# ElesionKyrie/Extreme-Video-Compression-With-Prediction-Using-Pre-trainded-Diffusion-Models-

Measured on AMD Instinct MI355X. Metric: decoded frames/sec (128x128x30) at q3, higher is better.
Workload: dtype f32

## Files before the change

extreme-video-compression-with-prediction-using-pre-trainded-diffusion-models-_amd/build.py:

```python
import os
import shutil
import subprocess
import sys
from concurrent.futures import ThreadPoolExecutor

HERE = os.path.dirname(os.path.abspath(__file__))
CSRC = os.path.join(HERE, "csrc")
LIBDIR = os.path.join(HERE, "lib")
OBJDIR = os.path.join(HERE, "build")
INCLUDE = os.path.join(os.path.dirname(HERE), "include")
HIP_SOURCES = ["conv_igemm.hip", "attention.hip", "norm.hip", "fir.hip", "elementwise.hip", "gdn.hip", "stride2.hip", "lpips.hip", "i3d.hip", "frames.hip", "noise.hip", "yuv.hip", "rate.hip", "ssim.hip", "api.hip"]
ARCH = "gfx950"


def _newer(target, deps):
    if not os.path.exists(target):
        return True
    t = os.path.getmtime(target)
    return any(os.path.getmtime(d) > t for d in deps)


def _run(cmd):
    r = subprocess.run(cmd, capture_output=True, text=True)
    if r.returncode != 0:
        raise RuntimeError("build failed: %s\n%s\n%s" % (" ".join(cmd), r.stdout, r.stderr))


def hipcc_path():
    for c in (os.environ.get("HIPCC"), shutil.which("hipcc"), "/opt/rocm/bin/hipcc"):
        if c and os.path.exists(c):
            return c
    raise RuntimeError("hipcc not found (ROCm toolchain required to build libevc_hip.so)")


def build(force=False, verbose=False):
    os.makedirs(LIBDIR, exist_ok=True)
    os.makedirs(OBJDIR, exist_ok=True)
    headers = [os.path.join(INCLUDE, h) for h in ("evc_hip.h", "evc_rans.h")]
    hipcc = hipcc_path()
    flags = ["--offload-arch=" + ARCH, "-O3", "-std=c++17", "-fPIC", "-I", INCLUDE]
    flags += os.environ.get("EVC_HIPCC_FLAGS", "").split()

    def compile_one(src):
        s = os.path.join(CSRC, src)
        o = os.path.join(OBJDIR, src.replace(".hip", ".o"))
        if force or _newer(o, [s] + headers):
            if verbose:
                print("hipcc", src, flush=True)
            _run([hipcc] + flags + ["-c", s, "-o", o])
        return o

    with ThreadPoolExecutor(max_workers=min(6, len(HIP_SOURCES))) as ex:
        objs = list(ex.map(compile_one, HIP_SOURCES))
    hip_so = os.path.join(LIBDIR, "libevc_hip.so")
    if force or _newer(hip_so, objs):
        _run([hipcc, "--offload-arch=" + ARCH, "-shared", "-fPIC", "-o", hip_so] + objs)
    rans_src = os.path.join(CSRC, "rans.cpp")
    rans_so = os.path.join(LIBDIR, "libevc_rans.so")
    if force or _newer(rans_so, [rans_src] + headers):
        _run([shutil.which("g++") or "g++", "-O2", "-std=c++17", "-fPIC", "-shared", "-Wall", "-I", INCLUDE,
              rans_src, "-o", rans_so])
    return hip_so, rans_so


# ... 3 lines not shown
```

extreme-video-compression-with-prediction-using-pre-trainded-diffusion-models-_amd/lib.py:

```python
import ctypes
import os
from ctypes import POINTER, c_char_p, c_double, c_float, c_int, c_int32, c_longlong, c_uint, c_uint8, c_ulonglong, c_void_p

import numpy as np
import torch

HERE = os.path.dirname(os.path.abspath(__file__))
HIP_SO = os.path.join(HERE, "lib", "libevc_hip.so")
if os.environ.get("EVC_HIP_SO"):
    HIP_SO = os.path.abspath(os.environ["EVC_HIP_SO"])
RANS_SO = os.path.join(HERE, "lib", "libevc_rans.so")

ACT_NONE, ACT_SILU, ACT_RELU = 0, 1, 2
ARITH_F32, ARITH_BF16X6, ARITH_F16X3 = 0, 1, 2
_ARITH_NAMES = {"f32": ARITH_F32, "bf16x6": ARITH_BF16X6, "f16x3": ARITH_F16X3}
_ARITH_DTYPES = {ARITH_F32: torch.float32, ARITH_BF16X6: torch.bfloat16, ARITH_F16X3: torch.float16}


def _arith_policy():
    name = os.environ.get("EVC_CONV_ARITH", "f16x3").lower()
    if name not in _ARITH_NAMES:
        raise ValueError(f"EVC_CONV_ARITH must be one of {sorted(_ARITH_NAMES)}, got {name!r}")
    return _ARITH_NAMES[name]

# ... 61 lines not shown
                                  c_void_p]),
    "evc_gn_coeffs_bound_f32": (c_int, [c_void_p, c_int, c_int, c_void_p, c_int, c_int, c_int, c_int, c_int, c_float,
                                        c_int, c_void_p, c_void_p, c_void_p, c_int, c_void_p, c_void_p, c_void_p,
                                        c_void_p, c_void_p, c_void_p]),
    "evc_moments_bound_f32": (c_int, [c_void_p, c_int, c_int, c_int, c_int, c_int, c_int, c_void_p, c_void_p, c_void_p]),
    "evc_gn_coeffs_site_f32": (c_int, [c_void_p, c_int, c_int, c_void_p, c_int, c_int, c_int, c_int, c_int, c_float,
                                       c_int, c_void_p, c_void_p, c_void_p, c_int, c_void_p, c_void_p, c_void_p,
                                       c_void_p, c_void_p, c_int, c_void_p]),
    "evc_gn_coeffs_bound_site_f32": (c_int, [c_void_p, c_int, c_int, c_void_p, c_int, c_int, c_int, c_int, c_int, c_float,
                                             c_int, c_void_p, c_void_p, c_void_p, c_int, c_void_p, c_void_p, c_void_p,
                                             c_void_p, c_void_p, c_void_p, c_int, c_void_p]),
    "evc_moments_bound_site_f32": (c_int, [c_void_p, c_int, c_int, c_int, c_int, c_int, c_int, c_void_p, c_void_p, c_void_p,
                                           c_int, c_void_p]),
    "evc_invariant_plan_revision": (c_int, []),
    "evc_conv_plan_query": (c_int, [POINTER(ConvArgs), POINTER(ConvPlan)]),
    "evc_gn_coeffs_bound_sample_f32": (c_int, [c_void_p, c_int, c_int, c_void_p, c_int, c_int, c_int, c_int, c_int, c_float,
                                               c_int, c_void_p, c_void_p, c_void_p, c_int, c_void_p, c_void_p, c_void_p,
                                               c_void_p, c_void_p, c_void_p, c_int, c_void_p]),
    "evc_moments_bound_sample_f32": (c_int, [c_void_p, c_int, c_int, c_int, c_int, c_int, c_int, c_void_p, c_void_p, c_void_p,
                                             c_int, c_void_p]),
    "evc_attention_invariant_workspace_bytes": (c_longlong, [c_int, c_int, c_int, c_int]),
    "evc_attention_invariant_f32": (c_int, [c_void_p, c_void_p, c_void_p, c_int, c_void_p, c_int, c_int, c_int, c_int, c_int,
                                            c_float, c_void_p, c_void_p, c_void_p]),
    "evc_attention_f16x3_f32": (c_int, [c_void_p, c_void_p, c_void_p, c_int, c_void_p, c_int, c_int, c_int, c_int, c_int,
                                        c_float, c_void_p, c_void_p, c_void_p]),
    "evc_deconv5x5s2_phase_weights_f32": (c_int, [c_void_p, c_void_p, c_int, c_int, c_int, c_int, c_void_p]),
    "evc_conv5x5s2_phase_weights_f32": (c_int, [c_void_p, c_void_p, c_int, c_int, c_int, c_void_p]),
    "evc_depth_to_space2_f32": (c_int, [c_void_p, c_int, c_int, c_void_p, c_int, c_int, c_int, c_int, c_void_p]),
    "evc_space_to_depth2_f32": (c_int, [c_void_p, c_int, c_int, c_void_p, c_int, c_int, c_int, c_int, c_int, c_void_p]),
    "evc_deconv5x5s2_workspace_bytes": (c_longlong, [c_int, c_int, c_int, c_int]),
    "evc_deconv5x5s2_f32": (c_int, [c_void_p, c_void_p, c_int, c_void_p, c_void_p, c_void_p] + [c_int] * 6 + [c_void_p]),
    "evc_conv5x5s2_workspace_bytes": (c_longlong, [c_int, c_int, c_int, c_int]),
    "evc_conv5x5s2_f32": (c_int, [c_void_p, c_int, c_void_p, c_int, c_void_p, c_void_p, c_void_p] + [c_int] * 6 + [c_void_p]),
    "evc_gdn_workspace_bytes": (c_longlong, [c_int, c_int, c_int, c_int]),
    "evc_gdn_f32": (c_int, [c_void_p, c_void_p, c_int, c_void_p, c_void_p, c_void_p, c_int, c_int, c_int, c_int, c_int,
                            c_int, c_void_p]),
    "evc_affine_act_nhwc_f32": (c_int, [c_void_p, c_void_p, c_void_p, c_void_p, c_int, c_int, c_int, c_int, c_int,
                                        c_int, c_void_p]),
    "evc_conv_co_pad": (c_int, [c_int]),
    "evc_conv_packed_floats": (c_longlong, [c_int, c_int, c_int, c_int]),
    "evc_conv_pack_weights_f32": (c_int, [c_void_p, c_void_p, c_int, c_int, c_int, c_int, c_void_p]),
    "evc_conv_packed_bytes": (c_longlong, [c_int, c_int, c_int, c_int, c_int]),
    "evc_conv_pack_weights": (c_int, [c_void_p, c_void_p, c_int, c_int, c_int, c_int, c_int, c_void_p]),
    "evc_conv_set_option": (c_int, [c_char_p, c_int]),
    "evc_spade_act_nhwc_f32": (c_int, [c_void_p, c_void_p, c_void_p, c_void_p, c_int, c_void_p, c_void_p, c_int, c_void_p,
                                       c_void_p, c_int, c_void_p, c_int, c_int, c_int, c_int, c_int, c_void_p]),
    "evc_conv_choose_splits": (c_int, [POINTER(ConvArgs)]),
    "evc_conv_kernel_name": (c_int, [POINTER(ConvArgs), c_char_p, c_int]),
    "evc_conv_fused_1x1_supported": (c_int, [POINTER(ConvArgs)]),
    "evc_conv_stats_splits": (c_int, [POINTER(ConvArgs)]),
    "evc_conv_workspace_bytes": (c_longlong, [POINTER(ConvArgs)]),
    "evc_conv2d_nhwc_f32": (c_int, [POINTER(ConvArgs), c_void_p, c_void_p]),
    "evc_conv2d_nhwc_profiled_f32": (c_int, [POINTER(ConvArgs), c_void_p, c_void_p, c_void_p, c_void_p]),
    "evc_attention_f32": (c_int, [c_void_p, c_void_p, c_void_p, c_int, c_void_p, c_int, c_int, c_int, c_int, c_int,
                                  c_float, c_void_p]),
    "evc_attention_workspace_bytes": (c_longlong, [c_int, c_int, c_int, c_int]),
    "evc_attention_set_option": (c_int, [c_char_p, c_int]),
    "evc_attention_ws_f32": (c_int, [c_void_p, c_void_p, c_void_p, c_int, c_void_p, c_int, c_int, c_int, c_int, c_int,
                                     c_float, c_void_p, c_void_p]),
    "evc_frame_group_norm_f32": (c_int, [c_void_p] * 4 + [c_int] * 5 + [c_float, c_void_p]),
    "evc_frame_attention_f32": (c_int, [c_void_p, c_int, c_void_p, c_int] + [c_int] * 5 + [c_float, c_void_p]),
    "evc_frame_mix_f32": (c_int, [c_void_p] * 4 + [c_int] * 3 + [c_longlong, c_void_p]),
    "evc_frame_taps_f32": (c_int, [c_void_p, c_void_p] + [c_int] * 4 + [c_void_p]),
    "evc_ddpm_step_f32": (c_int, [c_void_p, c_void_p, c_void_p, c_longlong] + [c_float] * 5 + [c_int, c_void_p]),
    "evc_ddim_step_f32": (c_int, [c_void_p, c_void_p, c_longlong] + [c_float] * 4 + [c_int, c_void_p]),
    "evc_axpy_f32": (c_int, [c_void_p, c_void_p, c_void_p, c_longlong, c_float, c_void_p]),
    "evc_pndm_transfer_f32": (c_int, [c_void_p, c_void_p, c_void_p, c_longlong, c_float, c_float, c_float, c_int,
                                      c_void_p]),
    "evc_lincomb4_f32": (c_int, [c_void_p] * 5 + [c_longlong] + [c_float] * 4 + [c_void_p]),
    "evc_scale_clamp_f32": (c_int, [c_void_p, c_void_p, c_longlong, c_float, c_float, c_int, c_float, c_float,
                                    c_void_p]),
    "evc_gate_residual_f32": (c_int, [c_void_p, c_void_p, c_void_p, c_void_p, c_longlong, c_void_p]),
    "evc_elic_gather_params_f32": (c_int, [c_void_p] + [c_int] * 8 + [c_void_p, c_int, c_void_p, c_void_p,
                                                                       c_void_p]),
    "evc_elic_scatter_symbols_f32": (c_int, [c_void_p, c_void_p, c_void_p] + [c_int] * 7 + [c_void_p]),
    "evc_elic_quantize_f32": (c_int, [c_void_p, c_int, c_int, c_void_p] + [c_int] * 5 + [c_void_p, c_void_p]),
    "evc_elic_rate_pass_f32": (c_int, [c_void_p] + [c_int] * 4 + [c_void_p] + [c_int] * 6 + [c_void_p, c_void_p, c_void_p]),
    "evc_bottleneck_rate_f32": (c_int, [c_void_p] + [c_int] * 5 + [c_void_p] * 5),
    "evc_noise_normal_f32": (c_int, [c_void_p, c_void_p, c_int, c_longlong, c_ulonglong, c_uint, c_int, c_void_p]),
    "evc_yuv420_to_rgb": (c_int, [c_void_p] + [c_longlong] * 6 + [c_int] * 5 + [c_void_p, c_int, c_void_p]),
    "evc_rgb_to_yuv420": (c_int, [c_void_p, c_void_p] + [c_longlong] * 6 + [c_int] * 4 + [c_void_p, c_void_p]),
    "evc_ssim_workspace_bytes": (c_longlong, [c_int, c_int, c_int]),
    "evc_ssim_planes_f32": (c_int, [c_void_p, c_void_p, c_int, c_int, c_int, c_void_p, c_double, c_double, c_void_p, c_void_p,
                                    c_void_p]),
}

RANS_SYMBOLS = {
    "evc_rans_version": (c_char_p, []),
    "evc_rans_max_encoded_bytes": (c_longlong, [c_longlong]),
    "evc_rans_encode_with_indexes": (c_longlong, [POINTER(c_int32), POINTER(c_int32), c_longlong, POINTER(c_int32),
                                                  c_int, POINTER(c_int32), POINTER(c_int32), c_int,
                                                  POINTER(c_uint8), c_longlong]),
    "evc_rans_decode_with_indexes": (c_int, [POINTER(c_uint8), c_longlong, POINTER(c_int32), c_longlong,
                                             POINTER(c_int32), c_int, POINTER(c_int32), POINTER(c_int32), c_int,
                                             POINTER(c_int32)]),
    "evc_pmf_to_quantized_cdf": (c_int, [POINTER(c_float), c_int, c_int, POINTER(c_int32)]),
}

_hip = None
_rans = None


def _load(path, symbols, what):
    if not os.path.exists(path):
        raise EvcLibraryError(f"{what} not built: {path} is missing. Run `python -c \"import __graft_entry__ as g; "
                              f"g.build()\"` (needs hipcc / g++). There is no fallback path.")
    lib = ctypes.CDLL(path)
    for name, (res, args) in symbols.items():
        try:
            fn = getattr(lib, name)
        except AttributeError as e:
            raise EvcLibraryError(f"{path} does not export {name}") from e
        fn.restype = res
        fn.argtypes = args
    return lib


def hip_lib(require_device=True):
    global _hip
    if _hip is None:
        _hip = _load(HIP_SO, HIP_SYMBOLS, "libevc_hip.so")
        for item in filter(None, os.environ.get("EVC_CONV_OPTIONS", "").split(",")):
            name, _, value = item.partition("=")
            if _hip.evc_conv_set_option(name.strip().encode(), int(value or 1)) != 0:
                raise ValueError(f"EVC_CONV_OPTIONS: unknown convolution option {name!r}")
    if require_device:
        if not torch.cuda.is_available():
            raise EvcLibraryError("no HIP device visible: the evc_amd compute path is gfx950-only (no CPU fallback)")
        if not getattr(hip_lib, "_checked", False):
            if _hip.evc_device_ok() != 1:
                raise EvcLibraryError("current HIP device is not gfx950 (MI355X); libevc_hip.so has no code for it")
            hip_lib._checked = True
    return _hip


def rans_lib():
    global _rans
    if _rans is None:
        _rans = _load(RANS_SO, RANS_SYMBOLS, "libevc_rans.so")
    return _rans


def _check(rc, name):
    if rc != 0:
        raise EvcKernelError(f"{name} failed with code {rc} "
                             "(-1 invalid argument, -2 unsupported, -3 launch failure)")


def stream_ptr():
    return c_void_p(torch.cuda.current_stream().cuda_stream)


def ptr(t):
    if t is None:
        return None
    assert t.is_cuda and t.is_contiguous(), "device-contiguous tensor required"
    return c_void_p(t.data_ptr())


def fptr(t, dtype=torch.float32):
    assert t is None or t.dtype == dtype, (t.dtype, dtype)
    return ptr(t)



def upfirdn2d_nchw(x, kernel, up=1, down=1, pad=(0, 0)):
    L = hip_lib()
    assert x.dim() == 4 and x.dtype == torch.float32
    x = x.contiguous()
    n, c, h, w = x.shape
    k = np.ascontiguousarray(np.asarray(kernel.detach().cpu() if torch.is_tensor(kernel) else kernel,
                                        dtype=np.float32))
    kh, kw = k.shape
    oh = (h * up + pad[0] + pad[1] - kh) // down + 1
    ow = (w * up + pad[0] + pad[1] - kw) // down + 1
    out = torch.empty((n, c, oh, ow), device=x.device, dtype=torch.float32)
    _check(L.evc_upfirdn2d_f32(fptr(x), fptr(out), k.ctypes.data_as(POINTER(c_float)), n * c, h, w, kh, kw, up, up,
                               down, down, pad[0], pad[1], pad[0], pad[1], stream_ptr()), "evc_upfirdn2d_f32")
# ... 445 lines not shown
    dev = (src0.t if isinstance(src0, Cols) else src0).device
    if out is None:
        out = torch.empty((B, H, W, Co), device=dev, dtype=torch.float32)
    po, Cout, ldo, shpo = _src(out)
    assert tuple(shpo) == (B, H, W) and Cout >= Co
    ca, cs = coef if coef is not None else (None, None)
    a = ConvArgs(p0, p1, C0, C1, ld0, ld1, ptr(ca), ptr(cs), act_in, ptr(w_packed), ptr(bias), ptr(res),
                 0 if res is None else res.shape[-1], float(out_scale), act_out, po, ldo,
                 B, H, W, Co, KH, KW, splits, None, packed_arith(w_packed), _word(in_bound, B if inv else 1))
    a.invariant = int(inv)
    x2_ci = 0
    if x2 is not None:
        q0, qC0, qld0, qshp = _src(x2[0])
        q1, qC1, qld1, _ = _src(x2[1])
        assert tuple(qshp) == (B, H, W) and x2[2].dtype == torch.float16
        a.x2_src0, a.x2_src1, a.x2_C0, a.x2_C1, a.x2_ld0, a.x2_ld1 = q0, q1, qC0, qC1, qld0, qld1
        a.x2_w_packed, a.x2_bound = ptr(x2[2]), _word(x2[3], B if inv else 1)
        x2_ci = qC0 + qC1
    stats = None
    if want_stats:
        ns = L.evc_conv_stats_splits(ctypes.byref(a))
        if ns > 0:
            stats = torch.empty((B, ns, Co, 2), device=dev, dtype=torch.float32)
            a.stats_out = ptr(stats)
    nbytes = L.evc_conv_workspace_bytes(ctypes.byref(a))
    if nbytes < 0:
        raise EvcKernelError(f"evc_conv_workspace_bytes rejected the arguments ({nbytes})")
    ws = _workspace(nbytes, dev) if nbytes > 0 else None
    if CONV_PROFILE is not None:
        st = torch.cuda.current_stream()
        e0, ec, e1 = (torch.cuda.Event(enable_timing=True) for _ in range(3))
        e0.record(st); ec.record(st)
        _check(L.evc_conv2d_nhwc_profiled_f32(ctypes.byref(a), ptr(ws), stream_ptr(), c_void_p(e0.cuda_event),
                                              c_void_p(ec.cuda_event)), "evc_conv2d_nhwc_profiled_f32")
        e1.record(st)
        kbuf = ctypes.create_string_buffer(96)
        L.evc_conv_kernel_name(ctypes.byref(a), kbuf, 96)
        CONV_PROFILE.append(dict(variant=conv_variant(Co), split=nbytes > 0, e0=e0, ec=ec, e1=e1, arith=a.arith,
                                 kernel=kbuf.value.decode(),
                                 flops=2.0 * B * H * W * Co * (KH * KW * (C0 + C1) + x2_ci),
                                 shape=(B, H, W, C0 + C1, Co, KH),
                                 call=dict(B=B, H=H, W=W, C0=C0, C1=C1, Co=Co, K=KH, coef=coef is not None, act_in=act_in,
                                           res=res is not None, out_scale=float(out_scale), bias=bias is not None,
                                           bound=in_bound is not None, arith=a.arith, ld_out=ldo,
                                           stats=bool(want_stats), x2=x2_ci, invariant=inv)))
    else:
        _check(L.evc_conv2d_nhwc_f32(ctypes.byref(a), ptr(ws), stream_ptr()), "evc_conv2d_nhwc_f32")
    result = out.t if isinstance(out, Cols) else out
    if want_stats:
        return result, (stats if stats is not None else chan_stats(result, invariant=inv))
    return result


def conv_fused_stats_splits(B, H, W, Ci, Co, KH, KW, splits=0, arith=None):
    a = conv_query_args(B, H, W, Ci, 0, Co, KH, KW, default_arith() if arith is None else arith, splits=splits)
    return hip_lib(require_device=False).evc_conv_stats_splits(ctypes.byref(a))


def conv_workspace_bytes(B, H, W, Ci, Co, KH, KW, splits=0, arith=None):
    a = conv_query_args(B, H, W, Ci, 0, Co, KH, KW, default_arith() if arith is None else arith, splits=splits)
    return hip_lib(require_device=False).evc_conv_workspace_bytes(ctypes.byref(a))


def attention_set_option(name, value):
    if hip_lib().evc_attention_set_option(name.encode(), int(value)) != 0:
        raise EvcKernelError(f"unknown attention option {name!r}")


def attention(qkv, C, heads, out=None, bounds=None, invariant=False):
    L = hip_lib()
    B, N, ld = qkv.shape
    D = C // heads
    if out is None:
        out = torch.empty((B, N, C), device=qkv.device, dtype=torch.float32)
    base = qkv.data_ptr()
    if bool(invariant):
        nbytes = L.evc_attention_invariant_workspace_bytes(B, heads, N, D)
        ws = _workspace(nbytes, qkv.device) if nbytes > 0 else None
        _check(L.evc_attention_invariant_f32(c_void_p(base), c_void_p(base + 4 * C), c_void_p(base + 8 * C), ld, fptr(out), C,
                                             B, heads, N, D, float(int(D) ** (-0.5)),
                                             None if bounds is None else _word(bounds, 3 * B), ptr(ws), stream_ptr()),
               "evc_attention_invariant_f32")
        return out
    nbytes = L.evc_attention_workspace_bytes(B, heads, N, D)
    ws = _workspace(nbytes, qkv.device) if nbytes > 0 else None
    if bounds is not None:
        _check(L.evc_attention_f16x3_f32(c_void_p(base), c_void_p(base + 4 * C), c_void_p(base + 8 * C), ld, fptr(out), C,
                                         B, heads, N, D, float(int(D) ** (-0.5)), _word(bounds, 3), ptr(ws), stream_ptr()),
               "evc_attention_f16x3_f32")
        return out
    _check(L.evc_attention_ws_f32(c_void_p(base), c_void_p(base + 4 * C), c_void_p(base + 8 * C), ld, fptr(out), C, B,
                                  heads, N, D, float(int(D) ** (-0.5)), ptr(ws), stream_ptr()), "evc_attention_ws_f32")
    return out


def frame_group_norm(x, N, gamma, beta, groups, eps):
    BN, H, W, C = x.shape
    assert BN % N == 0 and x.is_contiguous()
    y = torch.empty_like(x)
    _check(hip_lib().evc_frame_group_norm_f32(fptr(x), fptr(y), fptr(gamma), fptr(beta), BN // N, N, H * W, C, groups,
                                              float(eps), stream_ptr()), "evc_frame_group_norm_f32")
    return y


def frame_attention(qkv, N, C, heads):
    BN, H, W, ld = qkv.shape
# ... 322 lines not shown
```

extreme-video-compression-with-prediction-using-pre-trainded-diffusion-models-_amd/scorenet.py:

```python
import math
from types import SimpleNamespace

import numpy as np
import torch

from . import lib as L

FIR_K = np.outer([1, 3, 3, 1], [1, 3, 3, 1]).astype(np.float32)
FIR_K /= FIR_K.sum()
INV_SQRT2 = float(np.float32(1.0) / np.sqrt(np.float32(2.0)))


def num_groups(ch):
    g = min(ch // 4, 32)
    while ch % g != 0:
        g -= 1
    return g


def dims_from_config(config):
    m, d = config.model, config.data
    return SimpleNamespace(ngf=m.ngf, ch_mult=list(m.ch_mult), num_res_blocks=m.num_res_blocks,
                           attn_resolutions=list(m.attn_resolutions), n_head_channels=m.n_head_channels,
                           image_size=d.image_size, channels=d.channels, num_frames=d.num_frames,
# ... 152 lines not shown
        L.hip_lib()
        self.preactivate = preactivate
        self.config = config
        self.device = torch.device(device)
        self.d = dims_from_config(config)
        self.type = getattr(config.model, "type", "v1")
        m = config.model
        if bool(getattr(m, "spade", False)) != self.SPADE or getattr(m, "output_all_frames", False) or m.arch != self.ARCH:
            raise NotImplementedError("built: arch=unetmore -- the concat-conditioned network of configs/mine.yml (ScoreNet) and its "
                                      "SPADE variant (SpadeScoreNet) -- and arch=unetmorepseudo3d / unetmore3d without SPADE "
                                      "(Pseudo3dScoreNet / Conv3dScoreNet), all without output_all_frames (which fails in the "
                                      "reference itself: ncsnpp_more.py:384-385 splits 15 channels into 6 + 15)")
        self.cond_emb = bool(getattr(m, "cond_emb", False))
        self._init_wrapper(m, self.d.sigma_begin, self.d.sigma_end, self.d.num_classes)
        if self.batch_invariant and self.noise_in_cond:
            raise NotImplementedError("batch_invariant with noise_in_cond: the conditioning noise is drawn per batch")
        if (self.cond_emb or self.noise_in_cond) and self.SPADE:
            raise NotImplementedError("cond_emb / noise_in_cond are built for the concat-conditioned network only")
        self.embed_dim = self._embed_dim()
        self.program = self._build_program()
        if self.SPADE:
            self.program[2]["cin"] = self.d.channels * self.d.num_frames
        self._wsrc = {}
        self._load(state_dict, prefix + "unet.all_modules.")
        self.sites = range_sites(self.program, self.cond_emb) if self.RANGE_SITES else []
        self.site_words = L.site_word_arena(len(self.sites), self.device)
        self._demoted = set()
        self._attn_f32 = set()
        self._unfused = set()
        self._site_of = {}
        self._set_site_args()
        self.demote_seconds = 0.0
        self._rows = {}
        self._row_tensors = {}
        self._table = torch.zeros((256, self.ss_total), device=self.device, dtype=torch.float32)
        self._n_rows = 0
        self.use_graphs = use_graphs
        self._graphs = {}
        self._f16_raw = L.bounded_arith() == L.ARITH_F16X3
        import os
        self.overlap_skip = os.environ.get("EVC_OVERLAP_SKIP", "1") != "0"
        self.fuse_skip = self._f16_raw and os.environ.get("EVC_FUSE_SKIP", "1") != "0"
        self._side_streams = {}
        self._bounds_by_stream = {}
        self._bounds = None
        self._bound_next = 0
        self._bound_batch = 1
        if demote:
            self.demote(demote)

    def _conv(self, *a, **kw):
        return L.conv2d_nhwc(*a, invariant=self.batch_invariant, **kw)

    def _act(self, t, stats=None):
        return _Act(t, stats, invariant=self.batch_invariant)

    def _gn(self, *a, **kw):
        return L.gn_coeffs(*a, invariant=self.batch_invariant, **kw)

    def _mbound(self, *a, **kw):
        return L.moments_bound(*a, invariant=self.batch_invariant, **kw)

    def _attention(self, *a, **kw):
        return L.attention(*a, invariant=self.batch_invariant, **kw)

    def _fuse_ok(self, *a, **kw):
        return L.conv_fused_1x1_supported(*a, invariant=self.batch_invariant, **kw)

    def invariant_view(self):
        import copy
        if self.batch_invariant:
            return self
        if self.SPADE or self.ARCH != "unetmore" or self.noise_in_cond:
            raise NotImplementedError("batch_invariant is built for the concat-conditioned score network (ScoreNet) only")
        if self._demoted:
            raise ValueError("batch-invariant mode does not combine with demoted sites (range recovery)")
        v = copy.copy(self)
        v.batch_invariant = True
        v.taps = None
        v._rows, v._row_tensors = {}, {}
        v._table = torch.zeros_like(self._table)
        v._n_rows = 0
        v._graphs, v._side_streams, v._bounds_by_stream = {}, {}, {}
        v._bounds, v._bound_next = None, 0
        return v

    def _set_site_args(self):
        self._site_of = {(st["tag"], st["module"]): L.Site(self.site_words, st["site"], quiet=st["site"] in self._demoted)
                         for st in self.sites}

    def _site(self, tag, i):
        return self._site_of.get((tag, i))

    def _site_ids(self, sites):
        by_name = {st["name"]: st["site"] for st in self.sites}
        out = []
        for s in sites:
            k = by_name.get(s) if isinstance(s, str) else int(s)
            if k is None or not 0 <= k < len(self.sites):
                raise KeyError(f"no range-event site {s!r} in this network")
            out.append(k)
        return out

    def demote(self, sites):
        import time
        if self.batch_invariant:
# ... 204 lines not shown
            xs = torch.empty((B, Ho, Wo, m["cin"] if fuse else m["cout"]), device=self.device, dtype=torch.float32)
            side.wait_stream(main)
            with torch.cuda.stream(side):
                if fuse:
                    L.upfirdn2d_nhwc(x.t, *fir, out=xs)
                else:
                    skip_path(xs)
                done = torch.cuda.Event()
                done.record(side)
        if fir is not None:
            hf = L.upfirdn2d_nhwc(x.t, *fir, coef=coef0, act=L.ACT_SILU)
            h1 = self._act(*self._conv(hf, e["w0"], m["cout"], 3, 3, bias=e["b0"], want_stats=True))
        elif self.preactivate:
            cin = m["cin"]
            act = torch.empty((B, H, W, cin), device=self.device, dtype=torch.float32)
            c0 = x.t.shape[3]
            L.affine_act(x.t, coef0, L.ACT_SILU, out=L.Cols(act, 0, c0))
            if skip is not None:
                L.affine_act(skip.t, coef0, L.ACT_SILU, out=L.Cols(act, c0, cin - c0), coef_col=c0)
            h1 = self._act(*self._conv(act, e["w0"], m["cout"], 3, 3, bias=e["b0"], want_stats=True))
        else:
            h1 = self._act(*self._conv(x.t, e["w0"], m["cout"], 3, 3, bias=e["b0"], src1=s1, coef=coef0, act_in=L.ACT_SILU,
                                     want_stats=True))
        H1, W1 = h1.t.shape[1], h1.t.shape[2]
        coef1 = self._adagn([h1.stats()], H1 * W1, m["cout"], e["ss1"], rows, site=self._site("res1", i))
        if side is None:
            if fuse:
                xs = L.upfirdn2d_nhwc(x.t, *fir) if fir is not None else None
            else:
                xs = skip_path(None)
        else:
            torch.cuda.current_stream().wait_event(done)
        if fuse:
            x2 = (xs, None, e["w2"], xbound) if xs is not None else (x.t, s1, e["w2"], xbound)
            return self._act(*self._conv(h1.t, e["w1"], m["cout"], 3, 3, bias=e["b12"], coef=coef1, act_in=L.ACT_SILU,
                                       out_scale=INV_SQRT2, want_stats=True, x2=x2))
        if self.preactivate:
            h1a = L.affine_act(h1.t, coef1, L.ACT_SILU)
            return self._act(*self._conv(h1a, e["w1"], m["cout"], 3, 3, bias=e["b1"], res=xs, out_scale=INV_SQRT2,
                                       want_stats=True))
        return self._act(*self._conv(h1.t, e["w1"], m["cout"], 3, 3, bias=e["b1"], coef=coef1, act_in=L.ACT_SILU,
                                   res=xs, out_scale=INV_SQRT2, want_stats=True))

    def _attn(self, i, m, x):
        e = self.w[i]
        B, H, W, C = x.t.shape
        hd = self.d.n_head_channels
        heads = 1 if C < hd else C // hd
        coef = self._gn([x.stats()], H * W, num_groups(C), 1e-6, mode=1, gamma=e["gamma"], beta=e["beta"],
                           site=self._site("attn_norm", i))
        qkvb = self._bound_slot(3)
        if qkvb is None:
            obound = None
            qkv = self._conv(x.t, e["wqkv"], 3 * C, 1, 1, bias=e["bqkv"], coef=coef)
        else:
            qkv, qst = self._conv(x.t, e["wqkv"], 3 * C, 1, 1, bias=e["bqkv"], coef=coef, want_stats=True)
            self._mbound(qst, 0, C, qkvb, site=self._site("attn_qkv", i))
            obound = _f16_only(e["wo"], qkvb.view(B, 3)[:, 2].contiguous() if self.batch_invariant else qkvb[2:3])
        o = self._attention(qkv.view(B, H * W, 3 * C), C, heads, bounds=None if i in self._attn_f32 else qkvb)
        return self._act(*self._conv(o.view(B, H, W, C), e["wo"], C, 1, 1, bias=e["bo"], res=x.t,
                                   out_scale=INV_SQRT2, want_stats=True, in_bound=obound))

    @torch.no_grad()
    def forward_rows(self, x, rows, cond=None):
        if self.batch_invariant and self._demoted:
            raise ValueError("batch-invariant mode does not combine with demoted sites (range recovery)")
        return self._forward_rows(x, rows, cond)

    def _forward_rows(self, x, rows, cond=None):
        d = self.d
        prog = self.program
        B, _, H, W = x.shape
        self._bound_batch = B if self.batch_invariant else 1
        nb = 256 * self._bound_batch
        if self._f16_raw:
            if torch.cuda.is_current_stream_capturing():
                self._bounds = torch.empty(nb, device=self.device, dtype=torch.int32)
            else:
                key = torch.cuda.current_stream().cuda_stream
                self._bounds = self._bounds_by_stream.get(key)
                if self._bounds is None or self._bounds.numel() != nb:
                    self._bounds = self._bounds_by_stream[key] = torch.empty(nb, device=self.device, dtype=torch.int32)
            self._bounds.zero_()
            self._bound_next = 0
        taps = getattr(self, "taps", None)

        def tap(idx, act):
            if taps is not None:
                taps[idx] = act.t[..., :prog[idx].get("cout", prog[idx].get("ch"))].permute(0, 3, 1, 2).contiguous()
            return act
        i = 2
        m = prog[i]
        xin = self._pack_input(x, cond, self.w[i]["cin_pad"])
        hs = [tap(i, self._act(*self._conv(xin, self.w[i]["w"], m["cout"], 3, 3, bias=self.w[i]["b"], want_stats=True)))]
        i += 1
        n_lvl = len(d.ch_mult)
        for lvl in range(n_lvl):
            for _ in range(d.num_res_blocks):
                h = tap(i, self._res(i, prog[i], hs[-1], None, rows)); i += 1
                if h.t.shape[2] in d.attn_resolutions:
                    h = tap(i, self._attn(i, prog[i], h)); i += 1
                hs.append(h)
            if lvl != n_lvl - 1:
                hs.append(tap(i, self._res(i, prog[i], hs[-1], None, rows))); i += 1
        h = hs[-1]
        h = tap(i, self._res(i, prog[i], h, None, rows)); i += 1
        h = tap(i, self._attn(i, prog[i], h)); i += 1
        h = tap(i, self._res(i, prog[i], h, None, rows)); i += 1
        for lvl in reversed(range(n_lvl)):
            for _ in range(d.num_res_blocks + 1):
                h = tap(i, self._res(i, prog[i], h, hs.pop(), rows)); i += 1
            if h.t.shape[2] in d.attn_resolutions:
                h = tap(i, self._attn(i, prog[i], h)); i += 1
# ... 91 lines not shown
```

include/evc_hip.h:

```cpp
#ifndef EVC_HIP_H
#define EVC_HIP_H

#ifdef __cplusplus
extern "C" {
#endif

#define EVC_OK 0
#define EVC_EINVAL (-1)
#define EVC_EUNSUPPORTED (-2)
#define EVC_ELAUNCH (-3)

#define EVC_ACT_NONE 0
#define EVC_ACT_SILU 1
#define EVC_ACT_RELU 2

#define EVC_ARITH_F32 0
#define EVC_ARITH_BF16X6 1
#define EVC_ARITH_F16X3 2

const char* evc_version(void);
const char* evc_arch(void);
int evc_device_ok(void);

int evc_clock_probe(unsigned long long* out2, int spin_us, const unsigned* stop, void* stream);
// ... 24 lines not shown
                            const float* ss, int ss_ld, const int* row, float* coef_a, float* coef_s,
                            unsigned* bound_bits, unsigned* events, void* stream);
int evc_moments_bound_f32(const float* part, int nsplit, int C, int c_begin, int c_count, int n_ranges, int B,
                          unsigned* bound_bits, unsigned* events, void* stream);

int evc_gn_coeffs_site_f32(const float* part0, int nsplit0, int C0, const float* part1, int nsplit1, int C1, int B,
                           int HW, int groups, float eps, int mode, const float* gamma, const float* beta,
                           const float* ss, int ss_ld, const int* row, float* coef_a, float* coef_s, unsigned* events,
                           unsigned* site_events, int site, void* stream);
int evc_gn_coeffs_bound_site_f32(const float* part0, int nsplit0, int C0, const float* part1, int nsplit1, int C1, int B,
                                 int HW, int groups, float eps, int mode, const float* gamma, const float* beta,
                                 const float* ss, int ss_ld, const int* row, float* coef_a, float* coef_s,
                                 unsigned* bound_bits, unsigned* events, unsigned* site_events, int site, void* stream);
int evc_moments_bound_site_f32(const float* part, int nsplit, int C, int c_begin, int c_count, int n_ranges, int B,
                               unsigned* bound_bits, unsigned* events, unsigned* site_events, int site, void* stream);

int evc_affine_act_nhwc_f32(const float* x, float* y, const float* coef_a, const float* coef_s, int act, int B,
                            int HW, int C, int ld_coef, int ld_out, void* stream);

int evc_spade_act_nhwc_f32(const float* x, float* y, const float* coef_a, const float* coef_s, int ld_coef,
                           const float* gmap, const float* bmap, int ld_map, const float* ss_scale,
                           const float* ss_shift, int ld_ss, const int* row, int act, int B, int HW, int C, int ld_out,
                           void* stream);

typedef struct {
    const float* src0; const float* src1; int C0; int C1;
    int ld0; int ld1;
    const float* coef_a; const float* coef_s; int act_in;
    const float* w_packed; const float* bias; const float* res; int ld_res;
    float out_scale; int act_out;
    float* out; int ld_out;
    int B; int H; int W; int Co; int KH; int KW;
    int splits;
    float* stats_out;
    int arith;
    const unsigned* in_bound;
    const float* x2_src0; const float* x2_src1; int x2_C0; int x2_C1; int x2_ld0; int x2_ld1;
    const float* x2_w_packed; const unsigned* x2_bound;
    int invariant;
} evc_conv_args;
int evc_conv_co_pad(int Co);
long long evc_conv_packed_floats(int Co, int Ci, int KH, int KW);
int evc_conv_pack_weights_f32(const float* w, float* packed, int Co, int Ci, int KH, int KW, void* stream);
long long evc_conv_packed_bytes(int Co, int Ci, int KH, int KW, int arith);
int evc_conv_pack_weights(const float* w, void* packed, int Co, int Ci, int KH, int KW, int arith, void* stream);
int evc_conv_set_option(const char* name, int value);
int evc_conv_kernel_name(const evc_conv_args* a, char* buf, int n);
int evc_conv_choose_splits(const evc_conv_args* a);
int evc_conv_fused_1x1_supported(const evc_conv_args* a);
int evc_conv_stats_splits(const evc_conv_args* a);
long long evc_conv_workspace_bytes(const evc_conv_args* a);
int evc_conv2d_nhwc_f32(const evc_conv_args* a, float* ws, void* stream);

#define EVC_INVARIANT_REF_BATCH 9
int evc_invariant_plan_revision(void);
typedef struct {
    char kernel[96];
    int tile_m, tile_n, splits, steps_per_split, cut_chunk, tail_tiles, tail_splits, stats_runs, fused_1x1;
} evc_conv_plan;
int evc_conv_plan_query(const evc_conv_args* a, evc_conv_plan* out);
int evc_gn_coeffs_bound_sample_f32(const float* part0, int nsplit0, int C0, const float* part1, int nsplit1, int C1, int B,
                                   int HW, int groups, float eps, int mode, const float* gamma, const float* beta,
                                   const float* ss, int ss_ld, const int* row, float* coef_a, float* coef_s,
                                   unsigned* bound_bits, unsigned* events, unsigned* site_events, int site, void* stream);
int evc_moments_bound_sample_f32(const float* part, int nsplit, int C, int c_begin, int c_count, int n_ranges, int B,
                                 unsigned* bound_bits, unsigned* events, unsigned* site_events, int site, void* stream);
long long evc_attention_invariant_workspace_bytes(int B, int heads, int N, int D);
int evc_attention_invariant_f32(const float* q, const float* k, const float* v, int ld_qkv, float* out, int ld_out, int B,
                                int heads, int N, int D, float scale, const unsigned* bounds, float* ws, void* stream);

int evc_conv2d_nhwc_profiled_f32(const evc_conv_args* a, float* ws, void* stream, void* ev_start, void* ev_conv_end);

int evc_attention_f32(const float* q, const float* k, const float* v, int ld_qkv, float* out, int ld_out, int B,
                      int heads, int N, int D, float scale, void* stream);
long long evc_attention_workspace_bytes(int B, int heads, int N, int D);
int evc_attention_set_option(const char* name, int value);
int evc_attention_ws_f32(const float* q, const float* k, const float* v, int ld_qkv, float* out, int ld_out, int B,
                         int heads, int N, int D, float scale, float* ws, void* stream);

int evc_attention_f16x3_f32(const float* q, const float* k, const float* v, int ld_qkv, float* out, int ld_out, int B,
                            int heads, int N, int D, float scale, const unsigned* bounds, float* ws, void* stream);

int evc_frame_group_norm_f32(const float* x, float* y, const float* gamma, const float* beta, int B, int N, int HW, int C,
                             int groups, float eps, void* stream);
int evc_frame_attention_f32(const float* qkv, int ld_qkv, float* out, int ld_out, int B, int N, int HW, int C, int heads,
                            float scale, void* stream);
int evc_frame_mix_f32(const float* x, float* y, const float* w, const float* bias, int B, int N, int M, long long inner,
                      void* stream);

int evc_frame_taps_f32(const float* x, float* y, int B, int N, int HW, int C, void* stream);

int evc_ddpm_step_f32(float* x, const float* e, const float* noise, long long n, float k1, float k2, float c1,
                      float c2, float sigma, int clip, void* stream);
int evc_ddim_step_f32(float* x, const float* e, long long n, float k1, float k2, float c1, float c2, int clip,
                      void* stream);
int evc_axpy_f32(const float* x, const float* e, float* y, long long n, float alpha, void* stream);
int evc_pndm_transfer_f32(const float* x, const float* e, float* y, long long n, float d, float cx, float ce,
                          int clip, void* stream);
int evc_lincomb4_f32(const float* e0, const float* e1, const float* e2, const float* e3, float* y, long long n,
                     float w0, float w1, float w2, float w3, void* stream);
int evc_scale_clamp_f32(const float* x, float* y, long long n, float mul, float add, int clamp, float lo, float hi,
                        void* stream);

int evc_gate_residual_f32(const float* a, const float* b, const float* x, float* out, long long n, void* stream);
int evc_elic_gather_params_f32(const float* ms, int ld, int mean_off, int scale_off, int C, int B, int H, int W,
                               int parity, const float* scale_table, int n_scales, int* idx, float* means,
// ... 67 lines not shown
```

Baseline: 37.92.

## Add dedicated f16x3 MFMA projection GEMM for attention qkv and output 1x1 convs

Adds a specialized 1x1-convolution GEMM kernel using 32x32x16 f16 MFMA with a split-f16 (three-product) scheme, double-buffered LDS, register-ring weight prefetch, and fused affine input, bias, residual, scaling and per-64-row stats. Attention qkv and output projections route to it when shapes and arith allow, falling back to the generic implicit-GEMM conv otherwise. It aims to cut overhead of the general conv path for these pointwise projections. Two shapes are excluded as slower, and an env var can disable it.

```diff
diff --git a/extreme-video-compression-with-prediction-using-pre-trainded-diffusion-models-_amd/build.py b/extreme-video-compression-with-prediction-using-pre-trainded-diffusion-models-_amd/build.py
--- a/extreme-video-compression-with-prediction-using-pre-trainded-diffusion-models-_amd/build.py
+++ b/extreme-video-compression-with-prediction-using-pre-trainded-diffusion-models-_amd/build.py
@@ -9,7 +9,7 @@
 LIBDIR = os.path.join(HERE, "lib")
 OBJDIR = os.path.join(HERE, "build")
 INCLUDE = os.path.join(os.path.dirname(HERE), "include")
-HIP_SOURCES = ["conv_igemm.hip", "attention.hip", "norm.hip", "fir.hip", "elementwise.hip", "gdn.hip", "stride2.hip", "lpips.hip", "i3d.hip", "frames.hip", "noise.hip", "yuv.hip", "rate.hip", "ssim.hip", "api.hip"]
+HIP_SOURCES = ["conv_igemm.hip", "proj_gemm.hip", "attention.hip", "norm.hip", "fir.hip", "elementwise.hip", "gdn.hip", "stride2.hip", "lpips.hip", "i3d.hip", "frames.hip", "noise.hip", "yuv.hip", "rate.hip", "ssim.hip", "api.hip"]
 ARCH = "gfx950"
 
 
diff --git a/extreme-video-compression-with-prediction-using-pre-trainded-diffusion-models-_amd/csrc/proj_gemm.hip b/extreme-video-compression-with-prediction-using-pre-trainded-diffusion-models-_amd/csrc/proj_gemm.hip
--- /dev/null
+++ b/extreme-video-compression-with-prediction-using-pre-trainded-diffusion-models-_amd/csrc/proj_gemm.hip
@@ -0,0 +1,348 @@
+#include <hip/hip_runtime.h>
+#include <stdint.h>
+#include <string.h>
+#include <type_traits>
+#include "../../include/evc_hip.h"
+
+namespace {
+
+typedef float f32x16 __attribute__((ext_vector_type(16)));
+typedef _Float16 f16x8 __attribute__((ext_vector_type(8)));
+
+constexpr int KC = 16;
+constexpr int GC = 4;
+constexpr int F16_HDR_BYTES = 256;
+constexpr float F16_ACT_SCALE = 8.0f;
+
+struct ProjK {
+    const float* a; int lda;
+    const float* coef_a; const float* coef_s;
+    const char* w;
+    const float* w_hdr;
+    const unsigned* in_bound;
+    const float* bias; const float* res; int ld_res;
+    float out_scale;
+    float* out; int ld_out;
+    float* stats;
+    int M, HW, K, nchunk, ngroup, Co;
+};
+
+__device__ __forceinline__ float bound_scale(unsigned bits) {
+    const float b = sqrtf(__uint_as_float(bits));
+    if (!(b < 3.0e38f)) return __builtin_nanf("");
+    return b > 0.f ? ldexpf(1.0f, 6 - ilogbf(b)) : 1.0f;
+}
+
+__device__ __forceinline__ void split2_f16(const float4& v0, const float4& v1, float xscale, f16x8& p1, f16x8& p2) {
+    const float x[8] = {v0.x, v0.y, v0.z, v0.w, v1.x, v1.y, v1.z, v1.w};
+#pragma unroll
+    for (int j = 0; j < 8; ++j) {
+        const float v = x[j] * xscale;
+        const _Float16 a = (_Float16)v;
+        p1[j] = a; p2[j] = (_Float16)(v - (float)a);
+    }
+}
+
+__device__ __forceinline__ float4 affine4(float4 v, const float4& a, const float4& s) {
+    v.x = v.x * a.x + s.x; v.y = v.y * a.y + s.y; v.z = v.z * a.z + s.z; v.w = v.w * a.w + s.w;
+    return v;
+}
+
+__device__ __forceinline__ float4 keep4(float4 v, bool ok) {
+    v.x = ok ? v.x : 0.f; v.y = ok ? v.y : 0.f; v.z = ok ? v.z : 0.f; v.w = ok ? v.w : 0.f;
+    return v;
+}
+
+template <int WM, int WN, int TN, bool AFFINE, bool RES, bool STATS>
+__global__ __launch_bounds__(64 * WM * WN, 2) void proj_gemm_kernel(ProjK p) {
+    constexpr int NT = 64 * WM * WN;
+    constexpr int BM = 64 * WM, BN = 32 * TN * WN;
+    constexpr int NU = 8 / WN;
+    constexpr int RPP = NT / 8;
+    constexpr int R = TN == 1 ? 8 : 2;
+    constexpr int D = R - 1;
+    constexpr int PS = BM * 32, QS = 2 * PS, BUF = GC * QS;
+    static_assert((2 * GC) % R == 0 && 64 % RPP == 0 && NU * RPP == BM, "ring slots and producer passes must be compile-time");
+    extern __shared__ __attribute__((aligned(16))) char smem_p[];
+
+    const int tid = threadIdx.x;
+    const int lane = tid & 63;
+    const int wave = __builtin_amdgcn_readfirstlane(tid >> 6);
+    const int wm = wave / WN, wn = wave % WN;
+    const int l31 = lane & 31, half = lane >> 5;
+    const int m0 = blockIdx.x * BM;
+    const int n0 = blockIdx.y * BN;
+
+    const int kh = tid & 1, pq = (tid >> 3) & 3;
+    const int prow = (tid >> 5) * 4 + ((tid >> 1) & 3);
+    unsigned aoff[NU];
+    int brow[WM];
+#pragma unroll
+    for (int u = 0; u < NU; ++u) aoff[u] = (unsigned)min(m0 + u * RPP + prow, p.M - 1) * (unsigned)p.lda;
+#pragma unroll
+    for (int r = 0; r < WM; ++r) brow[r] = min(m0 + 64 * r, p.M - 1) / p.HW;
+    const float xscale = F16_ACT_SCALE * (p.in_bound ? bound_scale(p.in_bound[0]) : 1.0f);
+
+    float4 areg[NU][2];
+    float4 ca[WM][2], cs[WM][2];
+    bool aok = false;
+    auto issue_a = [&](int g) {
+        const int c = g * GC + pq;
+        aok = c < p.nchunk;
+        const unsigned ko = (unsigned)(min(c, p.nchunk - 1) * KC + 8 * kh);
+#pragma unroll
+        for (int u = 0; u < NU; ++u) {
+            const float* s = p.a + aoff[u] + ko;
+            areg[u][0] = *reinterpret_cast<const float4*>(s);
+            areg[u][1] = *reinterpret_cast<const float4*>(s + 4);
+        }
+        if (AFFINE) {
+#pragma unroll
+            for (int r = 0; r < WM; ++r) {
+                const size_t o = (size_t)brow[r] * p.K + ko;
+                ca[r][0] = *reinterpret_cast<const float4*>(p.coef_a + o);
+                ca[r][1] = *reinterpret_cast<const float4*>(p.coef_a + o + 4);
+                cs[r][0] = *reinterpret_cast<const float4*>(p.coef_s + o);
+                cs[r][1] = *reinterpret_cast<const float4*>(p.coef_s + o + 4);
+            }
+        }
+    };
+    auto store_a = [&](int buf) {
+        char* A = smem_p + buf * BUF + pq * QS;
+#pragma unroll
+        for (int u = 0; u < NU; ++u) {
+            const int r = (u * RPP) / 64;
+            const int row = u * RPP + prow;
+            const int o = row * 32 + 16 * (kh ^ ((row >> 3) & 1));
+            float4 v0 = areg[u][0], v1 = areg[u][1];
+            if (AFFINE) { v0 = affine4(v0, ca[r][0], cs[r][0]); v1 = affine4(v1, ca[r][1], cs[r][1]); }
+            f16x8 h1, h2;
+            split2_f16(keep4(v0, aok), keep4(v1, aok), xscale, h1, h2);
+            *reinterpret_cast<f16x8*>(A + o) = h1;
+            *reinterpret_cast<f16x8*>(A + o + PS) = h2;
+        }
+    };
+
+    const int fr = l31 * 32 + 16 * (half ^ ((l31 >> 3) & 1));
+    const int a_rd = wm * 64 * 32 + fr;
+    const char* const wb = p.w + (size_t)(n0 + wn * 32 * TN) * 32 + fr;
+    const size_t wplane = (size_t)p.Co * 32;
+    f16x8 bfr[R][2][TN];
+    auto load_b = [&](f16x8 (&dst)[2][TN], int c) {
+        const char* s = wb + (size_t)min(c, p.nchunk - 1) * 2 * wplane;
+#pragma unroll
+        for (int q = 0; q < 2; ++q)
+#pragma unroll
+            for (int j = 0; j < TN; ++j) dst[q][j] = *reinterpret_cast<const f16x8*>(s + q * wplane + j * 32 * 32);
+    };
+
+    f32x16 tot[2][TN];
+#pragma unroll
+    for (int i = 0; i < 2; ++i)
+#pragma unroll
+        for (int j = 0; j < TN; ++j)
+#pragma unroll
+            for (int r = 0; r < 16; ++r) tot[i][j][r] = 0.f;
+
+    issue_a(0);
+#pragma unroll
+    for (int d = 0; d < D; ++d) load_b(bfr[d], d);
+    store_a(0);
+    issue_a(min(1, p.ngroup - 1));
+    __syncthreads();
+
+    auto group = [&](int g, auto par) {
+        constexpr int P = decltype(par)::value;
+        const char* Ab = smem_p + P * BUF + a_rd;
+        f32x16 acc[2][TN];
+#pragma unroll
+        for (int i = 0; i < 2; ++i)
+#pragma unroll
+            for (int j = 0; j < TN; ++j)
+#pragma unroll
+                for (int r = 0; r < 16; ++r) acc[i][j][r] = 0.f;
+#pragma unroll
+        for (int q = 0; q < GC; ++q) {
+            load_b(bfr[(P * GC + q + D) % R], g * GC + q + D);
+            f16x8 a[2][2];
+#pragma unroll
+            for (int pl = 0; pl < 2; ++pl)
+#pragma unroll
+                for (int i = 0; i < 2; ++i) a[i][pl] = *reinterpret_cast<const f16x8*>(Ab + q * QS + pl * PS + i * 32 * 32);
+#pragma unroll
+            for (int t = 0; t < 3; ++t) {
+                const int qa = t == 0 ? 1 : 0, qb = t == 1 ? 1 : 0;
+#pragma unroll
+                for (int i = 0; i < 2; ++i)
+#pragma unroll
+                    for (int j = 0; j < TN; ++j)
+                        acc[i][j] = __builtin_amdgcn_mfma_f32_32x32x16_f16(a[i][qa], bfr[(P * GC + q) % R][qb][j], acc[i][j], 0, 0, 0);
+            }
+            if (q == 0) {
+                __builtin_amdgcn_sched_barrier(0);
+                store_a(P ^ 1);
+                issue_a(min(g + 2, p.ngroup - 1));
+            }
+        }
+#pragma unroll
+        for (int i = 0; i < 2; ++i)
+#pragma unroll
+            for (int j = 0; j < TN; ++j) tot[i][j] += acc[i][j];
+        __syncthreads();
+    };
+    for (int g = 0; g < p.ngroup; g += 2) {
+        group(g, std::integral_constant<int, 0>{});
+        if (g + 1 < p.ngroup) group(g + 1, std::integral_constant<int, 1>{});
+    }
+
+    const int wave_m0 = m0 + wm * 64;
+    if (wave_m0 >= p.M) return;
+    const float ascale = p.w_hdr[0] / (p.in_bound ? bound_scale(p.in_bound[0]) : 1.0f);
+    const float oscale = p.out_scale;
+    const int mw = wave_m0 + 4 * half;
+    const int cw = n0 + wn * 32 * TN + l31;
+#pragma unroll
+    for (int j = 0; j < TN; ++j) {
+        const int co = cw + j * 32;
+        const float bias = p.bias ? p.bias[co] : 0.f;
+        float st_sum = 0.f, st_sq = 0.f;
+#pragma unroll
+        for (int i = 0; i < 2; ++i) {
+            const int mb = mw + i * 32;
+            float rv[16];
+#pragma unroll
+            for (int r = 0; r < 16; ++r) rv[r] = 0.f;
+            if (RES) {
+                const float* rp = p.res + (size_t)mb * p.ld_res + co;
+#pragma unroll
+                for (int r = 0; r < 16; ++r) rv[r] = rp[(size_t)((r & 3) + 8 * (r >> 2)) * p.ld_res];
+            }
+            float* o = p.out + (size_t)mb * p.ld_out + co;
+#pragma unroll
+            for (int r = 0; r < 16; ++r) {
+                const float v = (tot[i][j][r] * ascale + bias + rv[r]) * oscale;
+                o[(size_t)((r & 3) + 8 * (r >> 2)) * p.ld_out] = v;
+                if (STATS) { st_sum += v; st_sq += v * v; }
+            }
+        }
+        if (STATS) {
+            st_sum += __shfl_xor(st_sum, 32);
+            st_sq += __shfl_xor(st_sq, 32);
+            if (half == 0) {
+                float* sp = p.stats + ((size_t)(wave_m0 >> 6) * p.Co + co) * 2;
+                sp[0] = st_sum; sp[1] = st_sq;
+            }
+        }
+    }
+}
+
+
+struct Tile { int wm, wn, tn; };
+constexpr Tile TILES[] = {{1, 2, 1}, {2, 2, 1}};
+constexpr int NTILES = (int)(sizeof(TILES) / sizeof(TILES[0]));
+
+inline bool measured_slower(int K, int N) { return (K == 384 && N == 1152) || (K == 768 && N == 2304); }
+
+int g_enabled = 1;
+int g_tile = -1;
+
+struct ProjPlan { int tile; dim3 grid, block; size_t lds; ProjK k; };
+
+inline int tile_bm(const Tile& t) { return 64 * t.wm; }
+inline int tile_bn(const Tile& t) { return 32 * t.tn * t.wn; }
+
+int proj_resolve(const evc_conv_args* a, ProjPlan& pl) {
+    if (!a || !a->src0 || !a->w_packed || !a->out) return EVC_EINVAL;
+    if (a->B <= 0 || a->H <= 0 || a->W <= 0 || a->Co <= 0 || a->C0 <= 0) return EVC_EINVAL;
+    if ((a->coef_a == nullptr) != (a->coef_s == nullptr)) return EVC_EINVAL;
+    if (!g_enabled) return EVC_EUNSUPPORTED;
+    if (a->arith != EVC_ARITH_F16X3) return EVC_EUNSUPPORTED;
+    if (a->KH != 1 || a->KW != 1) return EVC_EUNSUPPORTED;
+    if (a->src1 || a->C1 != 0) return EVC_EUNSUPPORTED;
+    if (a->act_in != EVC_ACT_NONE || a->act_out != EVC_ACT_NONE) return EVC_EUNSUPPORTED;
+    if (a->x2_w_packed || a->invariant || a->splits > 1) return EVC_EUNSUPPORTED;
+    if (a->Co % 64 != 0 || a->C0 % KC != 0) return EVC_EUNSUPPORTED;
+    const long long HW = (long long)a->H * a->W, M = HW * a->B;
+    if (HW % 64 != 0) return EVC_EUNSUPPORTED;
+    const int lda = a->ld0 ? a->ld0 : a->C0, ldo = a->ld_out ? a->ld_out : a->Co, ldr = a->ld_res ? a->ld_res : a->Co;
+    if (lda < a->C0 || ldo < a->Co || (a->res && ldr < a->Co) || ((lda | ldo | ldr) & 3)) return EVC_EINVAL;
+    if (M * lda >= (1LL << 31) || M * ldo >= (1LL << 31) || M * ldr >= (1LL << 31)) return EVC_EUNSUPPORTED;
+
+    if (measured_slower(a->C0, a->Co)) return EVC_EUNSUPPORTED;
+    int tile = g_tile;
+    if (tile < 0) {
+        const long long wg64 = (M / 64) * (a->Co / 64), wg128 = ((M + 127) / 128) * (a->Co / 64);
+        tile = (wg128 >= 128 && wg64 < 512) ? 1 : 0;
+    }
+    const Tile& t = TILES[tile];
+    pl.tile = tile;
+    pl.grid = dim3((unsigned)((M + tile_bm(t) - 1) / tile_bm(t)), (unsigned)(a->Co / tile_bn(t)), 1);
+    pl.block = dim3(64 * t.wm * t.wn);
+    pl.lds = (size_t)2 * GC * 2 * tile_bm(t) * 32;
+    ProjK& k = pl.k;
+    k.a = a->src0; k.lda = lda;
+    k.coef_a = a->coef_a; k.coef_s = a->coef_s;
+    k.w = reinterpret_cast<const char*>(a->w_packed) + F16_HDR_BYTES;
+    k.w_hdr = a->w_packed;
+    k.in_bound = a->in_bound;
+    k.bias = a->bias; k.res = a->res; k.ld_res = ldr;
+    k.out_scale = a->out_scale;
+    k.out = a->out; k.ld_out = ldo;
+    k.stats = a->stats_out;
+    k.M = (int)M; k.HW = (int)HW; k.K = a->C0; k.nchunk = a->C0 / KC; k.ngroup = (k.nchunk + GC - 1) / GC; k.Co = a->Co;
+    return EVC_OK;
+}
+
+template <int WM, int WN, int TN>
+void proj_launch(const ProjPlan& pl, hipStream_t st) {
+    const ProjK& k = pl.k;
+#define EVC_PROJ(AF, RE, ST) hipLaunchKernelGGL((proj_gemm_kernel<WM, WN, TN, AF, RE, ST>), pl.grid, pl.block, pl.lds, st, k)
+#define EVC_PROJ_RS(AF)                                   \
+    do {                                                  \
+        if (k.res && k.stats) EVC_PROJ(AF, true, true);   \
+        else if (k.res) EVC_PROJ(AF, true, false);        \
+        else if (k.stats) EVC_PROJ(AF, false, true);      \
+        else EVC_PROJ(AF, false, false);                  \
+    } while (0)
+    if (k.coef_a) EVC_PROJ_RS(true);
+    else EVC_PROJ_RS(false);
+#undef EVC_PROJ_RS
+#undef EVC_PROJ
+}
+
+}
+
+extern "C" int evc_proj_gemm_set_option(const char* name, int value) {
+    if (!name) return EVC_EINVAL;
+    if (!strcmp(name, "proj_gemm")) { g_enabled = value != 0; return EVC_OK; }
+    if (!strcmp(name, "tile")) {
+        if (value < -1 || value >= NTILES) return EVC_EINVAL;
+        g_tile = value;
+        return EVC_OK;
+    }
+    return EVC_EINVAL;
+}
+
+extern "C" int evc_proj_gemm_supported(const evc_conv_args* a) {
+    ProjPlan pl;
+    return proj_resolve(a, pl);
+}
+
+extern "C" int evc_proj_gemm_tile(const evc_conv_args* a, int* tile_m, int* tile_n) {
+    ProjPlan pl;
+    const int rc = proj_resolve(a, pl);
+    if (rc != EVC_OK) return rc;
+    if (tile_m) *tile_m = tile_bm(TILES[pl.tile]);
+    if (tile_n) *tile_n = tile_bn(TILES[pl.tile]);
+    return EVC_OK;
+}
+
+extern "C" int evc_proj_gemm_f16x3_f32(const evc_conv_args* a, void* stream) {
+    ProjPlan pl;
+    const int rc = proj_resolve(a, pl);
+    if (rc != EVC_OK) return rc;
+    hipStream_t st = (hipStream_t)stream;
+    if (pl.tile == 0) proj_launch<1, 2, 1>(pl, st);
+    else proj_launch<2, 2, 1>(pl, st);
+    return hipGetLastError() == hipSuccess ? EVC_OK : EVC_ELAUNCH;
+}
diff --git a/extreme-video-compression-with-prediction-using-pre-trainded-diffusion-models-_amd/lib.py b/extreme-video-compression-with-prediction-using-pre-trainded-diffusion-models-_amd/lib.py
--- a/extreme-video-compression-with-prediction-using-pre-trainded-diffusion-models-_amd/lib.py
+++ b/extreme-video-compression-with-prediction-using-pre-trainded-diffusion-models-_amd/lib.py
@@ -137,6 +137,10 @@
     "evc_conv_workspace_bytes": (c_longlong, [POINTER(ConvArgs)]),
     "evc_conv2d_nhwc_f32": (c_int, [POINTER(ConvArgs), c_void_p, c_void_p]),
     "evc_conv2d_nhwc_profiled_f32": (c_int, [POINTER(ConvArgs), c_void_p, c_void_p, c_void_p, c_void_p]),
+    "evc_proj_gemm_set_option": (c_int, [c_char_p, c_int]),
+    "evc_proj_gemm_supported": (c_int, [POINTER(ConvArgs)]),
+    "evc_proj_gemm_tile": (c_int, [POINTER(ConvArgs), POINTER(c_int), POINTER(c_int)]),
+    "evc_proj_gemm_f16x3_f32": (c_int, [POINTER(ConvArgs), c_void_p]),
     "evc_attention_f32": (c_int, [c_void_p, c_void_p, c_void_p, c_int, c_void_p, c_int, c_int, c_int, c_int, c_int,
                                   c_float, c_void_p]),
     "evc_attention_workspace_bytes": (c_longlong, [c_int, c_int, c_int, c_int]),
@@ -209,6 +213,8 @@
             name, _, value = item.partition("=")
             if _hip.evc_conv_set_option(name.strip().encode(), int(value or 1)) != 0:
                 raise ValueError(f"EVC_CONV_OPTIONS: unknown convolution option {name!r}")
+        if os.environ.get("EVC_PROJ_GEMM", "1") == "0":
+            _hip.evc_proj_gemm_set_option(b"proj_gemm", 0)
     if require_device:
         if not torch.cuda.is_available():
             raise EvcLibraryError("no HIP device visible: the evc_amd compute path is gfx950-only (no CPU fallback)")
@@ -760,6 +766,55 @@
     return result
 
 
+def proj_gemm_set_option(name, value):
+    _check(hip_lib(require_device=False).evc_proj_gemm_set_option(name.encode(), int(value)), "evc_proj_gemm_set_option")
+
+
+def proj_gemm_query(B, H, W, Ci, Co, arith=ARITH_F16X3, **kw):
+    K = kw.pop("K", 1)
+    C1 = kw.pop("C1", 0)
+    bound = kw.pop("bound", False)
+    a = conv_query_args(B, H, W, Ci, C1, Co, K, K, arith, **kw)
+    if bound:
+        a.in_bound = c_void_p(16)
+    return int(hip_lib(require_device=False).evc_proj_gemm_supported(ctypes.byref(a)))
+
+
+def proj_gemm_supported(B, H, W, Ci, Co, arith=ARITH_F16X3, **kw):
+    return proj_gemm_query(B, H, W, Ci, Co, arith, **kw) == 0
+
+
+def proj_gemm_tile(B, H, W, Ci, Co):
+    a = conv_query_args(B, H, W, Ci, 0, Co, 1, 1, ARITH_F16X3)
+    tm, tn = c_int(0), c_int(0)
+    _check(hip_lib(require_device=False).evc_proj_gemm_tile(ctypes.byref(a), ctypes.byref(tm), ctypes.byref(tn)),
+           "evc_proj_gemm_tile")
+    return tm.value, tn.value
+
+
+def proj_gemm(src0, w_packed, Co, bias=None, coef=None, res=None, out_scale=1.0, out=None, want_stats=False,
+              in_bound=None):
+    L = hip_lib()
+    p0, C0, ld0, shp = _src(src0)
+    B, H, W = shp
+    dev = (src0.t if isinstance(src0, Cols) else src0).device
+    if out is None:
+        out = torch.empty((B, H, W, Co), device=dev, dtype=torch.float32)
+    po, Cout, ldo, shpo = _src(out)
+    assert tuple(shpo) == (B, H, W) and Cout >= Co
+    ca, cs = coef if coef is not None else (None, None)
+    a = ConvArgs(p0, None, C0, 0, ld0, 0, ptr(ca), ptr(cs), ACT_NONE, ptr(w_packed), ptr(bias), ptr(res),
+                 0 if res is None else res.shape[-1], float(out_scale), ACT_NONE, po, ldo,
+                 B, H, W, Co, 1, 1, 0, None, packed_arith(w_packed), _word(in_bound))
+    stats = None
+    if want_stats:
+        stats = torch.empty((B, H * W // 64, Co, 2), device=dev, dtype=torch.float32)
+        a.stats_out = ptr(stats)
+    _check(L.evc_proj_gemm_f16x3_f32(ctypes.byref(a), stream_ptr()), "evc_proj_gemm_f16x3_f32")
+    result = out.t if isinstance(out, Cols) else out
+    return (result, stats) if want_stats else result
+
+
 def conv_fused_stats_splits(B, H, W, Ci, Co, KH, KW, splits=0, arith=None):
     a = conv_query_args(B, H, W, Ci, 0, Co, KH, KW, default_arith() if arith is None else arith, splits=splits)
     return hip_lib(require_device=False).evc_conv_stats_splits(ctypes.byref(a))
diff --git a/extreme-video-compression-with-prediction-using-pre-trainded-diffusion-models-_amd/scorenet.py b/extreme-video-compression-with-prediction-using-pre-trainded-diffusion-models-_amd/scorenet.py
--- a/extreme-video-compression-with-prediction-using-pre-trainded-diffusion-models-_amd/scorenet.py
+++ b/extreme-video-compression-with-prediction-using-pre-trainded-diffusion-models-_amd/scorenet.py
@@ -228,6 +228,14 @@
     def _conv(self, *a, **kw):
         return L.conv2d_nhwc(*a, invariant=self.batch_invariant, **kw)
 
+    def _proj(self, src, w, Co, **kw):
+        B, H, W, C = src.shape
+        if (not self.batch_invariant and L.packed_arith(w) == L.ARITH_F16X3
+                and L.proj_gemm_supported(B, H, W, C, Co, coef=kw.get("coef") is not None,
+                                          bound=kw.get("in_bound") is not None)):
+            return L.proj_gemm(src, w, Co, **kw)
+        return self._conv(src, w, Co, 1, 1, **kw)
+
     def _act(self, t, stats=None):
         return _Act(t, stats, invariant=self.batch_invariant)
 
@@ -538,13 +546,13 @@
         qkvb = self._bound_slot(3)
         if qkvb is None:
             obound = None
-            qkv = self._conv(x.t, e["wqkv"], 3 * C, 1, 1, bias=e["bqkv"], coef=coef)
+            qkv = self._proj(x.t, e["wqkv"], 3 * C, bias=e["bqkv"], coef=coef)
         else:
-            qkv, qst = self._conv(x.t, e["wqkv"], 3 * C, 1, 1, bias=e["bqkv"], coef=coef, want_stats=True)
+            qkv, qst = self._proj(x.t, e["wqkv"], 3 * C, bias=e["bqkv"], coef=coef, want_stats=True)
             self._mbound(qst, 0, C, qkvb, site=self._site("attn_qkv", i))
             obound = _f16_only(e["wo"], qkvb.view(B, 3)[:, 2].contiguous() if self.batch_invariant else qkvb[2:3])
         o = self._attention(qkv.view(B, H * W, 3 * C), C, heads, bounds=None if i in self._attn_f32 else qkvb)
-        return self._act(*self._conv(o.view(B, H, W, C), e["wo"], C, 1, 1, bias=e["bo"], res=x.t,
+        return self._act(*self._proj(o.view(B, H, W, C), e["wo"], C, bias=e["bo"], res=x.t,
                                    out_scale=INV_SQRT2, want_stats=True, in_bound=obound))
 
     @torch.no_grad()
diff --git a/include/evc_hip.h b/include/evc_hip.h
--- a/include/evc_hip.h
+++ b/include/evc_hip.h
@@ -100,6 +100,11 @@
 long long evc_conv_workspace_bytes(const evc_conv_args* a);
 int evc_conv2d_nhwc_f32(const evc_conv_args* a, float* ws, void* stream);
 
+int evc_proj_gemm_set_option(const char* name, int value);
+int evc_proj_gemm_supported(const evc_conv_args* a);
+int evc_proj_gemm_tile(const evc_conv_args* a, int* tile_m, int* tile_n);
+int evc_proj_gemm_f16x3_f32(const evc_conv_args* a, void* stream);
+
 #define EVC_INVARIANT_REF_BATCH 9
 int evc_invariant_plan_revision(void);
 typedef struct {
```

Result: no change. 38.13, median of 6 (+0.6%).
